# DixianZhu/deBWT

Measured on AMD Instinct MI355X. Metric: Gbp/sec BWT build (30 Gbp synthetic DNA); bit-exact vs CPU ref; 1/2/4/8-GPU, higher is better.
Workload: dtype u64

## Files before the change

debwt_amd/_lib.py:

```python
import ctypes
import os
import subprocess

_HERE = os.path.dirname(os.path.abspath(__file__))
LIB_PATH = os.environ.get("DEBWT_HIP_LIB", os.path.join(_HERE, "libdebwt_hip.so"))
_lib = None


class DebwtConfig(ctypes.Structure):
    _fields_ = [("k", ctypes.c_int), ("device", ctypes.c_int), ("sort_algo", ctypes.c_int),
                ("reserved", ctypes.c_int)]


class DebwtPackedText(ctypes.Structure):
    _fields_ = [("words", ctypes.POINTER(ctypes.c_uint64)), ("nwords", ctypes.c_uint64), ("n", ctypes.c_uint64),
                ("sep", ctypes.POINTER(ctypes.c_uint64)), ("nrec", ctypes.c_uint64),
                ("seconds_read", ctypes.c_double), ("seconds_pack", ctypes.c_double)]


class DebwtStats(ctypes.Structure):
    _fields_ = ([(n, ctypes.c_uint64) for n in (
        "n", "nrec", "red_capacity", "blue_capacity", "blue_bound_num", "case3num", "sp_len",
        "special_branch_num", "n_main", "distinct_keys", "blue_large_blocks", "blue_max_block")] +
        [(n, ctypes.c_float) for n in (
# ... 265 lines not shown


class DebwtMultiStats(ctypes.Structure):
    _fields_ = [("n", ctypes.c_uint64), ("nrec", ctypes.c_uint64), ("ngpus", ctypes.c_uint32), ("rounds", ctypes.c_uint32),
                ("key_bytes_in", ctypes.c_uint64), ("blue_bytes_in", ctypes.c_uint64), ("ms_build", ctypes.c_float),
                ("key_mode", ctypes.c_uint32), ("exchange_backend", ctypes.c_uint32)]

    def as_dict(self):
        return {n: getattr(self, n) for n, _ in self._fields_}


SYMBOLS = [
    "debwt_create", "debwt_destroy", "debwt_strerror", "debwt_last_error", "debwt_load_text",
    "debwt_load_ascii", "debwt_kmer_sort_rle", "debwt_classify", "debwt_sp_generate", "debwt_blue_sort",
    "debwt_bwt_assemble", "debwt_build", "debwt_fetch_bwt", "debwt_bwt_device_ptr", "debwt_get_stats",
    "debwt_fetch_array", "debwt_kmer_count_sorted", "debwt_radix_sort_u64", "debwt_radix_sort_u64_range", "debwt_radix_pair_passes", "debwt_radix_bucket_passes", "debwt_radix_low_finishes", "debwt_verify_inverse",
    "debwt_shard_begin", "debwt_shard_histogram", "debwt_shard_set_range", "debwt_shard_classify_local",
    "debwt_shard_facts_export", "debwt_shard_classify_global", "debwt_shard_info", "debwt_shard_fetch",
    "debwt_shard_partition_keys", "debwt_shard_plan", "debwt_shard_ranges", "debwt_shard_sort_begin",
    "debwt_shard_sort_range", "debwt_shard_sort_end", "debwt_concat_rows", "debwt_shard_export", "debwt_census_words", "debwt_shard_sp_flags", "debwt_shard_sp_emit",
    "debwt_shard_sp_import", "debwt_shard_blue_route", "debwt_shard_blue_place", "debwt_set_range_cap", "debwt_pack_fasta", "debwt_free_packed", "debwt_load_fasta", "debwt_pack_fasta_opts", "debwt_load_fasta_opts", "debwt_fasta_text_bound", "debwt_host_release_hold", "debwt_special_digest", "debwt_bwt_census", "debwt_fetch_rows", "debwt_verify_device", "debwt_multi_create", "debwt_multi_destroy", "debwt_multi_last_error",
    "debwt_multi_load_text", "debwt_multi_load_fasta", "debwt_multi_build", "debwt_multi_fetch_bwt", "debwt_multi_get_stats",
    "debwt_multi_verify", "debwt_multi_shard", "debwt_pinned_alloc", "debwt_pinned_free", "debwt_shard_key_mode",
    "debwt_multi_set_key_mode", "debwt_special_compare", "debwt_build_to_host", "debwt_multi_set_exchange", "debwt_reserve",
    "debwt_multi_set_serial", "debwt_multi_get_shard_report", "debwt_multi_step_name", "debwt_get_config",
    "debwt_dump_reference_files", "debwt_shard_scratch",
    "debwt_fm_create", "debwt_fm_open", "debwt_fm_last_error", "debwt_fm_info_get", "debwt_fm_samples",
    "debwt_fm_record_starts", "debwt_fm_count", "debwt_fm_locate", "debwt_fm_destroy",
    "debwt_fm_search", "debwt_fm_search_stats_get", "debwt_fm_mems", "debwt_fm_mems_stats_get",
    "debwt_fm_attach_text", "debwt_fm_extend", "debwt_fm_extend_stats_get", "debwt_fm_cluster_seeds",
    "debwt_fm_map_defaults", "debwt_fm_map", "debwt_fm_map_stats_get",
# ... 59 lines not shown
    L.debwt_bwt_device_ptr.argtypes = [vp, ctypes.POINTER(vp)]
    L.debwt_get_stats.restype = ctypes.c_int
    L.debwt_get_stats.argtypes = [vp, ctypes.POINTER(DebwtStats)]
    L.debwt_fetch_array.restype = ctypes.c_int
    L.debwt_fetch_array.argtypes = [vp, ctypes.c_int, vp, ctypes.c_uint64, u64p]
    L.debwt_kmer_count_sorted.restype = ctypes.c_int
    L.debwt_kmer_count_sorted.argtypes = [vp, u64p, u64p, ctypes.c_uint64, u64p]
    L.debwt_radix_sort_u64.restype = ctypes.c_int
    L.debwt_radix_sort_u64.argtypes = [vp, vp, vp, ctypes.c_uint64, ctypes.c_int, ctypes.POINTER(ctypes.c_float)]
    L.debwt_radix_pair_passes.restype = ctypes.c_uint64
    L.debwt_radix_pair_passes.argtypes = []
    L.debwt_radix_bucket_passes.restype = ctypes.c_uint64
    L.debwt_radix_bucket_passes.argtypes = []
    L.debwt_radix_low_finishes.restype = ctypes.c_uint64
    L.debwt_radix_low_finishes.argtypes = []
    L.debwt_radix_sort_u64_range.restype = ctypes.c_int
    L.debwt_radix_sort_u64_range.argtypes = [vp, vp, vp, ctypes.c_uint64, ctypes.c_int, ctypes.c_uint64, ctypes.c_uint64,
                                             ctypes.POINTER(ctypes.c_float)]
    L.debwt_verify_inverse.restype = ctypes.c_int
    L.debwt_verify_inverse.argtypes = [u64p, ctypes.c_uint64, u64p, ctypes.c_uint64, ctypes.c_uint64,
                                       ctypes.POINTER(ctypes.c_uint8)]
    L.debwt_shard_begin.restype = ctypes.c_int
    L.debwt_shard_begin.argtypes = [vp, ctypes.c_int, ctypes.c_int]
    L.debwt_shard_histogram.restype = ctypes.c_int
    L.debwt_shard_histogram.argtypes = [vp, u64p]
    L.debwt_shard_set_range.restype = ctypes.c_int
    L.debwt_shard_set_range.argtypes = [vp, ctypes.c_uint32, ctypes.c_uint32, ctypes.c_uint64, ctypes.c_uint64]
    L.debwt_shard_classify_local.restype = ctypes.c_int
    L.debwt_shard_classify_local.argtypes = [vp, u64p, u64p, u64p]
    L.debwt_shard_facts_export.restype = ctypes.c_int
# ... 237 lines not shown
```

debwt_amd/csrc/debwt_hip.hip:

```cpp
#include "../../include/debwt_hip.h"

#include <hip/hip_runtime.h>

#include <algorithm>
#include <new>
#include <chrono>
#include <cmath>
#include <cstdio>
#include <cstring>
#include <atomic>
#include <string>
#include <thread>
#include <tuple>
#include <vector>

#include "radix_sort.h"
#include "special_host.h"
#include "fasta_host.h"
#include "gz_parallel.h"
#include "stage_kernels.h"
#include "special_kernels.h"
#include "verify_kernels.h"
#include "fm_kernels.h"
#include "fm_search_kernels.h"
// ... 83 lines not shown
    u64 *routed = nullptr;
    struct SubSlice { u64 g0, g1, S, B; };
    std::vector<SubSlice> sub;
    std::thread special_thread;
    bool special_running = false;
    u64 g0 = 0, g1 = 0;
    u64 S_local = 0, B_slice = 0, sp_off = 0;
    int hbits = 10, pbits = 13;
    bool mzfilter = false;
    int mzw = 16;
    bool mztable = false;
    bool abs32 = true;

    hipStream_t copy_stream = nullptr;
    hipEvent_t ev_copy = nullptr, ev_copy2 = nullptr;
    std::vector<u64> census;
    bool census_valid = false;
    hipEvent_t ev[8]{};
    hipEvent_t ev_pass[16][2]{};
    int n_pass_events = 0;
};

namespace {

#define HIPCHK(ctx, call)                                                                      \
    do {                                                                                       \
        hipError_t e_ = (call);                                                                \
        if (e_ != hipSuccess) {                                                                \
            (ctx)->err = std::string(#call) + ": " + hipGetErrorString(e_);                    \
            return e_ == hipErrorOutOfMemory ? DEBWT_ENOMEM : DEBWT_EDEVICE;                   \
        }                                                                                      \
    } while (0)

size_t reclaim(debwt_ctx *c, const DevBuf *keep) {
    if (!c->reclaim_ok) return 0;
    std::vector<DevBuf *> idle;
    if (c->stage >= ST_CLASSIFIED) {
        idle = {&c->keysB, &c->dk, &c->dstart, &c->rs_rle, &c->pflag};
        if (!c->exchange) idle.push_back(&c->keysA);
        c->sk = nullptr; c->routed = nullptr;
    } else {
        idle = {&c->htab, &c->mi_list, &c->qlist, &c->qwave, &c->blue_tmp, &c->ls_buf, &c->vidx, &c->vtmp, &c->large_k0,
                &c->large_en, &c->rowsym, &c->spn, &c->spsym, &c->rbits, &c->blue, &c->momask, &c->mimask};
    }
    size_t freed = 0;
    (void)hipStreamSynchronize(c->stream);
    for (DevBuf *b : idle)
        if (b != keep && b->p) { freed += b->cap; (void)hipFree(b->p); b->p = nullptr; b->cap = 0; }
    if (getenv("DEBWT_TRACE_ALLOC")) fprintf(stderr, "reclaim: %.2f GB of idle buffers released\n", freed / 1e9);
    return freed;
}

int ensure(debwt_ctx *c, DevBuf &b, size_t bytes) {
    if (bytes <= b.cap) return DEBWT_OK;
    static const bool trace = getenv("DEBWT_TRACE_ALLOC") != nullptr;
    const auto t0 = std::chrono::steady_clock::now();
    const size_t old = b.cap;
    if (b.p) { HIPCHK(c, hipStreamSynchronize(c->stream)); HIPCHK(c, hipFree(b.p)); b.p = nullptr; b.cap = 0; }
    const auto t1 = std::chrono::steady_clock::now();
    size_t want = bytes + bytes / 16 + 256;
    hipError_t me = hipMalloc(&b.p, want);
// ... 72 lines not shown
int sync_check(debwt_ctx *c) {
    HIPCHK(c, hipStreamSynchronize(c->stream));
    HIPCHK(c, hipGetLastError());
    return DEBWT_OK;
}

struct DrainOnError {
    debwt_ctx *c;
    bool armed = true;
    ~DrainOnError() {
        if (!armed) return;
        if (c->copy_stream) (void)hipStreamSynchronize(c->copy_stream);
        if (c->stream) (void)hipStreamSynchronize(c->stream);
    }
};

inline u32 grid_for(u64 n, u32 block) { return (u32)((n + block - 1) / block); }

RadixWorkspace radix_ws(debwt_ctx *c) {
    RadixWorkspace ws{};
    ws.counts = c->rs_counts.as<u32>();
    ws.over = c->rs_over.as<u32>();
    ws.h_over = c->h_over;
    ws.over_cap = c->rs_over.cap >= 48 ? (u32)std::min<size_t>((c->rs_over.cap - 32) / 16, 0xFFFFFFFFu) : 0;
    ws.skew_list = c->rs_skew.as<u32>();
    ws.pair = c->rs_pair.as<u32>();
    ws.pair_cap = c->rs_pair.cap;
    return ws;
}

// ... 21 lines not shown
}

}


static std::vector<DevBuf *> all_buffers(debwt_ctx *c) {
    return {&c->text, &c->sepbits, &c->sep, &c->keysA, &c->keysB, &c->rs_counts, &c->cp_counts, &c->dk,
            &c->dstart, &c->mchar, &c->head_keys, &c->facts, &c->facts_tmp, &c->red, &c->red_q,
            &c->mi_j0, &c->mi_freq, &c->bstart, &c->cursor, &c->blue, &c->spkey, &c->sprow, &c->spchr,
            &c->branch, &c->pflag, &c->spsym, &c->spn, &c->bwt, &c->hmask, &c->hash_rows, &c->dollar,
            &c->large_q, &c->large_k0, &c->large_en, &c->rowsym, &c->momask, &c->mimask, &c->rbits, &c->rs_over, &c->rs_skew, &c->rs_pair,
            &c->mi_list, &c->htab, &c->fact_work, &c->facts_all, &c->shard_hist, &c->dest_tab, &c->qbounds, &c->qcursor,
            &c->sx, &c->sppos, &c->sprec, &c->tail_d, &c->brbits,
            &c->blk_j0, &c->blk_freq, &c->blk_start, &c->facts_acc, &c->large_tmp, &c->blue_tmp, &c->sub_start, &c->sub_j0,
            &c->sub_freq, &c->sub_depth, &c->range_hist, &c->rs_rle, &c->ls_buf, &c->vidx, &c->vtmp, &c->qlist, &c->qwave,
            &c->blue_done};
}

extern "C" const char *debwt_strerror(int code) {
    switch (code) {
        case DEBWT_OK: return "ok";
        case DEBWT_EINVAL: return "invalid argument";
        case DEBWT_ENOMEM: return "out of memory";
        case DEBWT_EDEVICE: return "HIP runtime error";
        case DEBWT_ESTATE: return "stage called out of order";
        case DEBWT_ERANGE: return "input exceeds a capacity of this build";
        case DEBWT_EINTERNAL: return "internal consistency check failed";
        case DEBWT_EIO: return "file could not be written";
        default: return "unknown error";
    }
}
// ... 7 lines not shown
}

extern "C" int debwt_create(const debwt_config *cfg, debwt_ctx **out) {
    if (!cfg || !out || cfg->k < 12 || cfg->k > 32) return DEBWT_EINVAL;
    int ndev = 0;
    if (hipGetDeviceCount(&ndev) != hipSuccess || cfg->device < 0 || cfg->device >= ndev) return DEBWT_EDEVICE;
    debwt_ctx *c = new (std::nothrow) debwt_ctx();
    if (!c) return DEBWT_ENOMEM;
    c->cfg = *cfg;
    if (c->cfg.sort_algo == 0) c->cfg.sort_algo = 3;
    c->K = cfg->k - 1;
    int rc = DEBWT_OK;
    auto fail = [&](int code) { debwt_destroy(c); return code; };
    if (hipSetDevice(cfg->device) != hipSuccess) return fail(DEBWT_EDEVICE);
    if (hipStreamCreateWithFlags(&c->stream, hipStreamNonBlocking) != hipSuccess) return fail(DEBWT_EDEVICE);
    if (hipHostMalloc((void **)&c->h_scalars, 64 * sizeof(u32), hipHostMallocDefault) != hipSuccess)
        return fail(DEBWT_ENOMEM);
    for (auto &e : c->ev) if (hipEventCreate(&e) != hipSuccess) return fail(DEBWT_EDEVICE);
    for (auto &p : c->ev_pass) for (auto &e : p) if (hipEventCreate(&e) != hipSuccess) return fail(DEBWT_EDEVICE);
    if ((rc = ensure(c, c->rs_counts, radix_workspace_bytes(0))) != DEBWT_OK) return fail(rc);
    if ((rc = ensure(c, c->rs_over, radix_over_bytes(1 << 20))) != DEBWT_OK) return fail(rc);
    if (hipHostMalloc((void **)&c->h_over, 64, hipHostMallocDefault) != hipSuccess)
        return fail(DEBWT_ENOMEM);
    if ((rc = ensure(c, c->cp_counts, 8 * (CP_MAXCHUNKS + 16) * sizeof(u32))) != DEBWT_OK) return fail(rc);
    if ((rc = ensure(c, c->dollar, 64)) != DEBWT_OK) return fail(rc);
    *out = c;
    return DEBWT_OK;
}

extern "C" void debwt_destroy(debwt_ctx *c) {
    if (!c) return;
    if (c->special_running) { c->special_thread.join(); c->special_running = false; }
    (void)hipSetDevice(c->cfg.device);
    if (c->stream) (void)hipStreamSynchronize(c->stream);
    for (DevBuf *b : all_buffers(c)) if (b->p) (void)hipFree(b->p);
    if (c->h_scalars) (void)hipHostFree(c->h_scalars);
    if (c->h_over) (void)hipHostFree(c->h_over);
    for (auto &e : c->ev) if (e) (void)hipEventDestroy(e);
    for (auto &p : c->ev_pass) for (auto &e : p) if (e) (void)hipEventDestroy(e);
    if (c->ev_copy) (void)hipEventDestroy(c->ev_copy);
    if (c->ev_copy2) (void)hipEventDestroy(c->ev_copy2);
    if (c->copy_stream) { (void)hipStreamSynchronize(c->copy_stream); (void)hipStreamDestroy(c->copy_stream); }
    if (c->stream) (void)hipStreamDestroy(c->stream);
    delete c;
}

static void join_special(debwt_ctx *c);

extern "C" int debwt_load_text(debwt_ctx *c, const uint64_t *packed, uint64_t n, const uint64_t *sep, uint64_t nrec) {
    if (!c || !packed || !sep || nrec == 0 || n < 34) return DEBWT_EINVAL;
    join_special(c);
    if (sep[nrec - 1] != n - 1) return DEBWT_EINVAL;
    uint64_t prev = 0;
    for (uint64_t r = 0; r < nrec; r++) {
        uint64_t start = r ? sep[r - 1] + 1 : 0;
        if (sep[r] < start + 33 || sep[r] >= n) return DEBWT_EINVAL;
        prev = sep[r];
// ... 778 lines not shown
    ENSURE(c, c->htab, ht_slots * sizeof(HSlot));
    HIPCHK(c, hipMemsetAsync(c->rbits.p, 0, rb_bytes, c->stream));
    HIPCHK(c, hipMemsetAsync(c->htab.p, 0, ht_slots * sizeof(HSlot), c->stream));
    if (c->R) {
        k_build_hash<<<grid_for(c->R, 256), 256, 0, c->stream>>>(c->red.as<u64>(), c->R, c->red_q.as<u32>(),
                                                                c->blk_start.as<u64>(), c->abs32 ? 1 : 0, (u32)c->qbase,
                                                                (u32)c->Q, hbits, c->htab.as<HSlot>(), c->mzfilter ? 0 : pb,
                                                                c->rbits.as<u32>(), c->mztable ? c->K : 0);
        if (c->mzfilter)
            k_build_mzfilter<<<grid_for(c->R, 256), 256, 0, c->stream>>>(c->red.as<u64>(), c->R, c->K, pb, c->rbits.as<u64>(), c->mzw);
    }
    return DEBWT_OK;
}

#define SP_SLICE_GROUPS (1ull << 26)
static SpBlockIds sp_block_ids(debwt_ctx *c) {
    if (!c->route_direct) return SpBlockIds{nullptr, nullptr, nullptr, 0};
    return SpBlockIds{c->qlist.as<u32>(), c->qwave.as<unsigned long long>(), c->qwave.as<u64>() + 1, c->gq0};
}
static int sp_block_ids_begin(debwt_ctx *c, u64 gq0, u64 groups) {
    c->route_direct = true; c->gq0 = gq0;
    ENSURE(c, c->qlist, (std::min<u64>(groups * 32, c->Btotal) + 64) * 4);
    ENSURE(c, c->qwave, ((groups + 63) / 64 + 2) * 8);
    HIPCHK(c, hipMemsetAsync(c->qwave.p, 0, 8, c->stream));
    return DEBWT_OK;
}

static int sp_flags(debwt_ctx *c, u64 g0, u64 g1) {
    int rc;
    if (g1 - g0 > (1ull << 27) - 2) { c->err = "text slice of the SP stage exceeds 2^32 positions"; return DEBWT_ERANGE; }
    c->g0 = g0; c->g1 = g1;
    const u64 ng = g1 - g0;
    if (ng && c->mzfilter && c->mztable)
        k_sp_flags<2><<<grid_for(ng, DEBWT_BLOCK), DEBWT_BLOCK, 0, c->stream>>>(
            c->text.as<u64>(), c->sepbits.as<u64>(), c->n, c->K, c->htab.as<HSlot>(), c->hbits, c->rbits.as<u32>(), c->pbits,
            c->branch.as<u64>(), c->nbranch, c->momask.as<u32>(), c->mimask.as<u32>(), g0, g1,
            sp_block_ids(c), c->branch_bitmap ? c->brbits.as<u64>() : nullptr);
    else if (ng && c->mzfilter)
        k_sp_flags<1><<<grid_for(ng, DEBWT_BLOCK), DEBWT_BLOCK, 0, c->stream>>>(
            c->text.as<u64>(), c->sepbits.as<u64>(), c->n, c->K, c->htab.as<HSlot>(), c->hbits, c->rbits.as<u32>(), c->pbits,
            c->branch.as<u64>(), c->nbranch, c->momask.as<u32>(), c->mimask.as<u32>(), g0, g1,
            sp_block_ids(c), c->branch_bitmap ? c->brbits.as<u64>() : nullptr, c->mzw);
    else if (ng)
        k_sp_flags<0><<<grid_for(ng, DEBWT_BLOCK), DEBWT_BLOCK, 0, c->stream>>>(
            c->text.as<u64>(), c->sepbits.as<u64>(), c->n, c->K, c->htab.as<HSlot>(), c->hbits, c->rbits.as<u32>(), c->pbits,
            c->branch.as<u64>(), c->nbranch, c->momask.as<u32>(), c->mimask.as<u32>(), g0, g1,
            sp_block_ids(c), c->branch_bitmap ? c->brbits.as<u64>() : nullptr);
    SpCountF fc{c->momask.as<u32>() + g0, c->mimask.as<u32>() + g0};
    if ((rc = cp_count2(c, fc, ng, cp_area(c, 0), 8, cp_area(c, 1), 10))) return rc;
    if ((rc = sync_check(c))) return rc;
    c->S_local = c->h_scalars[8];
    c->B_slice = c->h_scalars[10];
    return DEBWT_OK;
}

static int sp_emit(debwt_ctx *c, u64 sp_off, u64 *routed = nullptr, int qshift = 0) {
    const u64 ng = c->g1 - c->g0;
    c->sp_off = sp_off;
    ENSURE_KEEP(c, c->spsym, sp_off + c->S_local + 64, c->shard_world > 1 ? 0 : sp_off);
    if (!routed) ENSURE(c, c->mi_list, c->B_slice * 16 + 64);
    if (ng) {
        SpEmitArgs ea{c->text.as<u64>(), c->sepbits.as<u64>(), c->n, c->K, c->momask.as<u32>(), c->mimask.as<u32>(),
                      c->spsym.as<u8>(), routed ? nullptr : c->mi_list.as<ulonglong2>(), c->g0, sp_off,
                      routed, qshift, sp_block_ids(c)};
        u32 nchunks; u64 chunk;
        plan_chunks(ng, &nchunks, &chunk);
        k_sp_emit<<<nchunks, DEBWT_BLOCK, 0, c->stream>>>(ea, ng, chunk, cp_area(c, 0), cp_area(c, 1));
    }
    return DEBWT_OK;
}

static int sp_finish(debwt_ctx *c, u64 S) {
    c->S = S;
    u64 ntriples = (S >> 6) + 3;
    ENSURE(c, c->spn, ntriples * 24);
    k_pack_sp<<<grid_for(ntriples, 256), 256, 0, c->stream>>>(c->spsym.as<u8>(), S, ntriples, c->spn.as<u64>());
    c->st.sp_len = S;
    c->stage = ST_SP;
    return DEBWT_OK;
}

extern "C" int debwt_sp_generate(debwt_ctx *c) {
// ... 14 lines not shown
                            !((c->cfg.reserved & 262144) && c->ranges.size() > 1);
    const size_t P = c->ranges.size();
    bool route_ranges = !route_sort && c->shard_world == 1 && P > 1 && P <= RS_RADIX && c->Q > 0 && c->n < (1ull << (qshift - 3)) &&
                        !(c->cfg.reserved & 32);
    for (size_t i = 0; route_ranges && i < P; i++) route_ranges = c->ranges[i].B < 0xFFFFFFF0ull - (1ull << 20);
    std::vector<u64> rfill(P, 0), roffs(P + 1, 0);
    if (route_ranges) {
        std::vector<u32> qb(P + 1);
        for (size_t i = 0; i < P; i++) qb[i] = (u32)c->ranges[i].qbase;
        qb[P] = (u32)c->Q;
        ENSURE(c, c->qbounds, (P + 1) * 4);
        HIPCHK(c, hipMemcpyAsync(c->qbounds.p, qb.data(), (P + 1) * 4, hipMemcpyHostToDevice, c->stream));
        HIPCHK(c, hipStreamSynchronize(c->stream));
    }
    c->route_direct = false;
    for (u64 g0 = 0; g0 < ngroups; g0 += slice_groups) {
        const u64 g1 = std::min(ngroups, g0 + slice_groups);
        if ((route_sort || route_ranges) && (rc = sp_block_ids_begin(c, g0, g1 - g0))) return rc;
        if ((rc = sp_flags(c, g0, g1))) return rc;
        if (route_sort) {
            if (Bseen + c->B_slice > c->B) { c->err = "multi-in positions exceed the block total"; return DEBWT_EINTERNAL; }
            if ((rc = sp_emit(c, S, c->blue.as<u64>() + Bseen, qshift))) return rc;
        } else if (route_ranges) {
            u64 *ta = c->keysA.as<u64>(), *tb = c->keysB.as<u64>();
            size_t tb_cap = c->keysB.cap / 8;
            if (c->keysA.cap < c->B_slice * 8 + 64) { ENSURE(c, c->blue_tmp, c->B_slice * 8 + 64); ta = c->blue_tmp.as<u64>(); }
            if (c->keysB.cap < c->B_slice * 8 + 64) { ENSURE(c, c->mi_list, c->B_slice * 8 + 64); tb = c->mi_list.as<u64>(); tb_cap = c->mi_list.cap / 8; }
            if ((rc = sp_emit(c, S, ta, qshift))) return rc;
            if (c->B_slice) {
                ENSURE(c, c->rs_over, radix_over_bytes(c->B_slice));
                RsDigit dg{};
// ... 218 lines not shown
}

static int blue_sort_part(debwt_ctx *c, const BlueQueue &bq, u64 q0, u64 nq, u64 l0, u64 nl) {
    int rc;
    if (!nq) return DEBWT_OK;
    const u32 Q = (u32)nq;
    const u64 *bst = c->blk_start.as<u64>() + q0, *bj0 = c->blk_j0.as<u64>() + q0;
    const u32 *bfr = c->blk_freq.as<u32>() + q0;
    const BlueSub &sub = bq.sub;
    const u32 sub_cap = bq.cap;
    u32 *sub_count = bq.count;
    HIPCHK(c, hipMemsetAsync(c->sub_freq.p, 0, (size_t)sub_cap * 4, c->stream));
    HIPCHK(c, hipMemsetAsync(sub_count, 0, 4, c->stream));
    BlueSub none{};
    u32 g1 = (u32)std::min<u64>(Q, 1u << 16);
    const u32 tiny = (c->cfg.reserved & 16777216) ? 0u : 2 * BLUE_TINY;
    if (tiny) {
        k_blue_tiny<16><<<g1, 64, 0, c->stream>>>(c->blue.as<u64>(), bst, bfr, bj0, Q, c->spn.as<u64>(), c->S, c->mchar.as<u8>(),
                                                  nullptr, nullptr);
        k_blue_tiny<32><<<g1, 64, 0, c->stream>>>(c->blue.as<u64>(), bst, bfr, bj0, Q, c->spn.as<u64>(), c->S, c->mchar.as<u8>(),
                                                  nullptr, nullptr);
    }
    k_blue_refine<64, 128, 0><<<g1, 64, 0, c->stream>>>(c->blue.as<u64>(), bst, bfr, bj0, Q, tiny,
                                                       c->spn.as<u64>(), c->S, c->mchar.as<u8>(), nullptr, nullptr, none);
    k_blue_refine<64, 256, 128><<<g1, 64, 0, c->stream>>>(c->blue.as<u64>(), bst, bfr, bj0, Q, 128u, c->spn.as<u64>(), c->S,
                                                         c->mchar.as<u8>(), nullptr, nullptr, sub);
    const bool split1024 = c->n1024 >= 1024;
    const bool by_classes = split1024 || c->n512 >= 1024;
    const u8 *done = nullptr;
    if ((by_classes || (c->cfg.reserved & 1048576)) && sub.cap && !(c->cfg.reserved & 524288)) {
        ENSURE(c, c->blue_done, c->Q + 64);
        u8 *dn = c->blue_done.as<u8>() + q0;
        HIPCHK(c, hipMemsetAsync(dn, 0, Q, c->stream));
        const u32 gc = (u32)std::min<u64>(Q, 1u << 14);
        k_blue_classify<BLUE_WAVE_CAP, BLUE_WAVE_CAP><<<gc, 256, 0, c->stream>>>(c->blue.as<u64>(), bst, bfr, bj0, Q, 256u, c->spn.as<u64>(),
                                                                                 c->S, c->mchar.as<u8>(), sub, dn);
        k_blue_classify<1024, BLUE_WAVE_CAP><<<gc, 256, 0, c->stream>>>(c->blue.as<u64>(), bst, bfr, bj0, Q, (u32)BLUE_WAVE_CAP,
                                                                        c->spn.as<u64>(), c->S, c->mchar.as<u8>(), sub, dn);
        k_blue_classify<BLUE_LDS_CAP, BLUE_WAVE_CAP><<<(u32)std::min<u64>(Q, 1u << 12), 256, 0, c->stream>>>(
            c->blue.as<u64>(), bst, bfr, bj0, Q, 1024u, c->spn.as<u64>(), c->S, c->mchar.as<u8>(), sub, dn);
        done = dn;
    }
    k_blue_refine<256, BLUE_WAVE_CAP, 128><<<(u32)std::min<u64>(Q, 1u << 14), 256, 0, c->stream>>>(
        c->blue.as<u64>(), bst, bfr, bj0, Q, 256u, c->spn.as<u64>(), c->S, c->mchar.as<u8>(), nullptr, nullptr, sub, done);
    u32 g2 = (u32)std::min<u64>(Q, 1u << 12);
    if (split1024)
        k_blue_refine<256, 1024, BLUE_WAVE_CAP><<<g2, 256, 0, c->stream>>>(c->blue.as<u64>(), bst, bfr, bj0, Q, (u32)BLUE_WAVE_CAP,
                                                                      c->spn.as<u64>(), c->S, c->mchar.as<u8>(), nullptr, nullptr, sub, done);
    k_blue_refine<256, BLUE_LDS_CAP, BLUE_WAVE_CAP><<<g2, 256, 0, c->stream>>>(c->blue.as<u64>(), bst, bfr, bj0, Q,
                                                                  split1024 ? 1024u : (u32)BLUE_WAVE_CAP, c->spn.as<u64>(), c->S,
                                                                  c->mchar.as<u8>(), nullptr, nullptr, sub, done);
    if (nl && (rc = sort_large_blocks(c, sub, l0, nl))) return rc;
    const u32 gs = std::min<u32>(sub_cap, 1u << 16);
    if (done) {
        u32 *snap = sub_count + 1;
        for (int level = 0; level < BLUE_QUEUE_LEVELS; level++) {
            k_copy_u32<<<1, 1, 0, c->stream>>>(sub_count, snap);
            k_blue_classify<BLUE_WAVE_CAP, BLUE_WAVE_CAP><<<std::min<u32>(gs, 1u << 14), 256, 0, c->stream>>>(
                c->blue.as<u64>(), c->sub_start.as<u64>(), c->sub_freq.as<u32>(), c->sub_j0.as<u64>(), sub_cap, 128u, c->spn.as<u64>(),
                c->S, c->mchar.as<u8>(), sub, nullptr, c->sub_depth.as<u32>(), snap, c->sub_freq.as<u32>());
        }
    }
    if (tiny) {
        k_blue_tiny<16><<<gs, 64, 0, c->stream>>>(c->blue.as<u64>(), c->sub_start.as<u64>(), c->sub_freq.as<u32>(), c->sub_j0.as<u64>(),
                                                  sub_cap, c->spn.as<u64>(), c->S, c->mchar.as<u8>(), c->sub_depth.as<u32>(), sub_count);
        k_blue_tiny<32><<<gs, 64, 0, c->stream>>>(c->blue.as<u64>(), c->sub_start.as<u64>(), c->sub_freq.as<u32>(), c->sub_j0.as<u64>(),
// ... 796 lines not shown
        std::vector<u32> first(D);
        HIPCHK(c, hipMemcpy(first.data(), c->dstart.p, D * 4, hipMemcpyDeviceToHost));
        for (u64 i = 0; i < ncopy; i++) counts[i] = (i + 1 < D ? first[i + 1] : (u32)Mk) - first[i];
    }
    return DEBWT_OK;
}

extern "C" int debwt_radix_sort_u64(debwt_ctx *c, uint64_t *d_keys, uint64_t *d_tmp, uint64_t count, int key_bits,
                                    float *ms_per_pass) {
    return debwt_radix_sort_u64_range(c, d_keys, d_tmp, count, key_bits, 0, 0, ms_per_pass);
}

extern "C" uint64_t debwt_radix_pair_passes(void) { return radix_pair_passes(); }
extern "C" uint64_t debwt_radix_bucket_passes(void) { return radix_bucket_passes(); }
extern "C" uint64_t debwt_radix_low_finishes(void) { return radix_low_finishes(); }

__global__ void k_keys_outside(const u64 *__restrict__ keys, u64 n, u64 lo, u64 hi, u32 *__restrict__ flag) {
    bool bad = false;
    for (u64 i = (u64)blockIdx.x * blockDim.x + threadIdx.x; i < n; i += (u64)gridDim.x * blockDim.x) bad |= keys[i] < lo || keys[i] > hi;
    if (bad) *flag = 1u;
}

extern "C" int debwt_radix_sort_u64_range(debwt_ctx *c, uint64_t *d_keys, uint64_t *d_tmp, uint64_t count, int key_bits,
                                          uint64_t key_lo, uint64_t key_hi, float *ms_per_pass) {
    if (!c || !d_keys || !d_tmp || key_bits < 1 || key_bits > 64) return DEBWT_EINVAL;
    if (key_hi && key_hi <= key_lo) return DEBWT_EINVAL;
    if (count >= 0xFFFFFFF0ull) return DEBWT_ERANGE;
    HIPCHK(c, hipSetDevice(c->cfg.device));
    ENSURE(c, c->rs_skew, (count / 2048 + 2) * 4);
    ENSURE(c, c->rs_over, radix_over_bytes(count));
// ... 4209 lines not shown
```

include/debwt_hip.h:

```cpp
#ifndef DEBWT_HIP_H
#define DEBWT_HIP_H
#include <stddef.h>
#include <stdint.h>
#ifdef __cplusplus
extern "C" {
#endif

#define DEBWT_OK 0
#define DEBWT_EINVAL (-1)
#define DEBWT_ENOMEM (-2)
#define DEBWT_EDEVICE (-3)
#define DEBWT_ESTATE (-4)
#define DEBWT_ERANGE (-5)
#define DEBWT_EINTERNAL (-6)
#define DEBWT_EIO (-7)

typedef struct debwt_ctx debwt_ctx;

typedef struct {
    int k;
    int device;
    int sort_algo;
    int reserved;
} debwt_config;
// ... 161 lines not shown
#define DEBWT_DUMP_BLOCKS 2
#define DEBWT_DUMP_SP 3
int debwt_dump_reference_files(debwt_ctx *ctx, const char *dir, int stage);


int debwt_kmer_count_sorted(debwt_ctx *ctx, uint64_t *kmers, uint64_t *counts, uint64_t capacity,
                            uint64_t *distinct);

int debwt_radix_sort_u64(debwt_ctx *ctx, uint64_t *d_keys, uint64_t *d_tmp, uint64_t count, int key_bits,
                         float *ms_per_pass);
int debwt_radix_sort_u64_range(debwt_ctx *ctx, uint64_t *d_keys, uint64_t *d_tmp, uint64_t count, int key_bits,
                               uint64_t key_lo, uint64_t key_hi, float *ms_per_pass);
uint64_t debwt_radix_pair_passes(void);
uint64_t debwt_radix_bucket_passes(void);
uint64_t debwt_radix_low_finishes(void);

int debwt_special_digest(const uint64_t *packed, uint64_t n, const uint64_t *sep, uint64_t nrec, int k, uint64_t digest[4]);

int debwt_special_compare(debwt_ctx *ctx, uint64_t mismatch[6]);

int debwt_verify_inverse(const uint64_t *bwt, uint64_t n, const uint64_t *hash_rows, uint64_t nrec,
                         uint64_t dollar_row, uint8_t *sym_out);

typedef struct {
    uint64_t segments, steps, mismatches, broken_links, search_failures, search_steps;
    float ms_index, ms_search, ms_walk;
    int ok;
} debwt_verify_report;
int debwt_verify_device(debwt_ctx *ctx, const uint64_t *d_words, const uint64_t *hash_rows, uint64_t dollar_row,
                        uint64_t segments, debwt_verify_report *report);
// ... 295 lines not shown
```

Before: 24.36.

## Overlap SP flag/emit slices and small blue-block refinement on an auxiliary stream

Adds an auxiliary HIP stream with fork/join events. The SP stage now double-buffers its per-slice block-id and count areas, so the flags of slice s+1 are computed on the main stream while slice s is emitted on the aux stream. The blue sort launches the tiny/small-block refinement kernels on the aux stream concurrently with the large-class classify/refine kernels on the main stream. The aim is to hide host sync gaps and let underutilizing small kernels run alongside each other, at the cost of extra buffers, more events, and some risk of races on shared sub-block counters.

```diff
diff --git a/debwt_amd/_lib.py b/debwt_amd/_lib.py
--- a/debwt_amd/_lib.py
+++ b/debwt_amd/_lib.py
@@ -303,7 +303,7 @@
     "debwt_create", "debwt_destroy", "debwt_strerror", "debwt_last_error", "debwt_load_text",
     "debwt_load_ascii", "debwt_kmer_sort_rle", "debwt_classify", "debwt_sp_generate", "debwt_blue_sort",
     "debwt_bwt_assemble", "debwt_build", "debwt_fetch_bwt", "debwt_bwt_device_ptr", "debwt_get_stats",
-    "debwt_fetch_array", "debwt_kmer_count_sorted", "debwt_radix_sort_u64", "debwt_radix_sort_u64_range", "debwt_radix_pair_passes", "debwt_radix_bucket_passes", "debwt_radix_low_finishes", "debwt_verify_inverse",
+    "debwt_fetch_array", "debwt_kmer_count_sorted", "debwt_radix_sort_u64", "debwt_radix_sort_u64_range", "debwt_radix_pair_passes", "debwt_radix_bucket_passes", "debwt_radix_low_finishes", "debwt_overlapped_launches", "debwt_verify_inverse",
     "debwt_shard_begin", "debwt_shard_histogram", "debwt_shard_set_range", "debwt_shard_classify_local",
     "debwt_shard_facts_export", "debwt_shard_classify_global", "debwt_shard_info", "debwt_shard_fetch",
     "debwt_shard_partition_keys", "debwt_shard_plan", "debwt_shard_ranges", "debwt_shard_sort_begin",
@@ -393,6 +393,8 @@
     L.debwt_radix_bucket_passes.argtypes = []
     L.debwt_radix_low_finishes.restype = ctypes.c_uint64
     L.debwt_radix_low_finishes.argtypes = []
+    L.debwt_overlapped_launches.restype = ctypes.c_uint64
+    L.debwt_overlapped_launches.argtypes = []
     L.debwt_radix_sort_u64_range.restype = ctypes.c_int
     L.debwt_radix_sort_u64_range.argtypes = [vp, vp, vp, ctypes.c_uint64, ctypes.c_int, ctypes.c_uint64, ctypes.c_uint64,
                                              ctypes.POINTER(ctypes.c_float)]
diff --git a/debwt_amd/csrc/debwt_hip.hip b/debwt_amd/csrc/debwt_hip.hip
--- a/debwt_amd/csrc/debwt_hip.hip
+++ b/debwt_amd/csrc/debwt_hip.hip
@@ -121,6 +121,12 @@
 
     hipStream_t copy_stream = nullptr;
     hipEvent_t ev_copy = nullptr, ev_copy2 = nullptr;
+    hipStream_t aux_stream = nullptr;
+    hipEvent_t ev_fork = nullptr, ev_join = nullptr, ev_totals[2]{}, ev_emit[2]{};
+    bool aux_busy = false;
+    DevBuf qwave2, qlist2;
+    u32 *qlist_b = nullptr;
+    u64 gq0_b = 0;
     std::vector<u64> census;
     bool census_valid = false;
     hipEvent_t ev[8]{};
@@ -147,11 +153,12 @@
         if (!c->exchange) idle.push_back(&c->keysA);
         c->sk = nullptr; c->routed = nullptr;
     } else {
-        idle = {&c->htab, &c->mi_list, &c->qlist, &c->qwave, &c->blue_tmp, &c->ls_buf, &c->vidx, &c->vtmp, &c->large_k0,
+        idle = {&c->htab, &c->mi_list, &c->qlist, &c->qwave, &c->qlist2, &c->qwave2, &c->blue_tmp, &c->ls_buf, &c->vidx, &c->vtmp, &c->large_k0,
                 &c->large_en, &c->rowsym, &c->spn, &c->spsym, &c->rbits, &c->blue, &c->momask, &c->mimask};
     }
     size_t freed = 0;
     (void)hipStreamSynchronize(c->stream);
+    if (c->aux_stream) (void)hipStreamSynchronize(c->aux_stream);
     for (DevBuf *b : idle)
         if (b != keep && b->p) { freed += b->cap; (void)hipFree(b->p); b->p = nullptr; b->cap = 0; }
     if (getenv("DEBWT_TRACE_ALLOC")) fprintf(stderr, "reclaim: %.2f GB of idle buffers released\n", freed / 1e9);
@@ -254,6 +261,39 @@
         if (c->stream) (void)hipStreamSynchronize(c->stream);
     }
 };
+
+enum { STREAMS_SP = 1, STREAMS_BLUE = 2 };
+std::atomic<u64> overlapped_launches{0};
+int streams_parts(const debwt_ctx *c) {
+    if (!c->aux_stream) return 0;
+    const char *e = getenv("DEBWT_STREAMS");
+    if (!e || !*e) return STREAMS_SP | STREAMS_BLUE;
+    if (!strcmp(e, "sp")) return STREAMS_SP;
+    if (!strcmp(e, "blue")) return STREAMS_BLUE;
+    return atoi(e) == 1 ? 0 : STREAMS_SP | STREAMS_BLUE;
+}
+int aux_fork(debwt_ctx *c) {
+    HIPCHK(c, hipEventRecord(c->ev_fork, c->stream));
+    HIPCHK(c, hipStreamWaitEvent(c->aux_stream, c->ev_fork, 0));
+    c->aux_busy = true;
+    return DEBWT_OK;
+}
+int aux_join(debwt_ctx *c) {
+    if (!c->aux_busy) return DEBWT_OK;
+    HIPCHK(c, hipEventRecord(c->ev_join, c->aux_stream));
+    HIPCHK(c, hipStreamWaitEvent(c->stream, c->ev_join, 0));
+    c->aux_busy = false;
+    return DEBWT_OK;
+}
+struct AuxDrain {
+    debwt_ctx *c;
+    ~AuxDrain() {
+        if (!c->aux_busy) return;
+        (void)hipStreamSynchronize(c->aux_stream);
+        c->aux_busy = false;
+    }
+};
+inline void aux_count(u64 n = 1) { overlapped_launches.fetch_add(n, std::memory_order_relaxed); }
 
 inline u32 grid_for(u64 n, u32 block) { return (u32)((n + block - 1) / block); }
 
@@ -305,7 +345,7 @@
             &c->sx, &c->sppos, &c->sprec, &c->tail_d, &c->brbits,
             &c->blk_j0, &c->blk_freq, &c->blk_start, &c->facts_acc, &c->large_tmp, &c->blue_tmp, &c->sub_start, &c->sub_j0,
             &c->sub_freq, &c->sub_depth, &c->range_hist, &c->rs_rle, &c->ls_buf, &c->vidx, &c->vtmp, &c->qlist, &c->qwave,
-            &c->blue_done};
+            &c->blue_done, &c->qwave2, &c->qlist2};
 }
 
 extern "C" const char *debwt_strerror(int code) {
@@ -343,6 +383,9 @@
     auto fail = [&](int code) { debwt_destroy(c); return code; };
     if (hipSetDevice(cfg->device) != hipSuccess) return fail(DEBWT_EDEVICE);
     if (hipStreamCreateWithFlags(&c->stream, hipStreamNonBlocking) != hipSuccess) return fail(DEBWT_EDEVICE);
+    if (hipStreamCreateWithFlags(&c->aux_stream, hipStreamNonBlocking) != hipSuccess) return fail(DEBWT_EDEVICE);
+    for (hipEvent_t *e : {&c->ev_fork, &c->ev_join, &c->ev_totals[0], &c->ev_totals[1], &c->ev_emit[0], &c->ev_emit[1]})
+        if (hipEventCreateWithFlags(e, hipEventDisableTiming) != hipSuccess) return fail(DEBWT_EDEVICE);
     if (hipHostMalloc((void **)&c->h_scalars, 64 * sizeof(u32), hipHostMallocDefault) != hipSuccess)
         return fail(DEBWT_ENOMEM);
     for (auto &e : c->ev) if (hipEventCreate(&e) != hipSuccess) return fail(DEBWT_EDEVICE);
@@ -351,7 +394,7 @@
     if ((rc = ensure(c, c->rs_over, radix_over_bytes(1 << 20))) != DEBWT_OK) return fail(rc);
     if (hipHostMalloc((void **)&c->h_over, 64, hipHostMallocDefault) != hipSuccess)
         return fail(DEBWT_ENOMEM);
-    if ((rc = ensure(c, c->cp_counts, 8 * (CP_MAXCHUNKS + 16) * sizeof(u32))) != DEBWT_OK) return fail(rc);
+    if ((rc = ensure(c, c->cp_counts, 10 * (CP_MAXCHUNKS + 16) * sizeof(u32))) != DEBWT_OK) return fail(rc);
     if ((rc = ensure(c, c->dollar, 64)) != DEBWT_OK) return fail(rc);
     *out = c;
     return DEBWT_OK;
@@ -362,6 +405,7 @@
     if (c->special_running) { c->special_thread.join(); c->special_running = false; }
     (void)hipSetDevice(c->cfg.device);
     if (c->stream) (void)hipStreamSynchronize(c->stream);
+    if (c->aux_stream) (void)hipStreamSynchronize(c->aux_stream);
     for (DevBuf *b : all_buffers(c)) if (b->p) (void)hipFree(b->p);
     if (c->h_scalars) (void)hipHostFree(c->h_scalars);
     if (c->h_over) (void)hipHostFree(c->h_over);
@@ -370,6 +414,8 @@
     if (c->ev_copy) (void)hipEventDestroy(c->ev_copy);
     if (c->ev_copy2) (void)hipEventDestroy(c->ev_copy2);
     if (c->copy_stream) { (void)hipStreamSynchronize(c->copy_stream); (void)hipStreamDestroy(c->copy_stream); }
+    for (hipEvent_t e : {c->ev_fork, c->ev_join, c->ev_totals[0], c->ev_totals[1], c->ev_emit[0], c->ev_emit[1]}) if (e) (void)hipEventDestroy(e);
+    if (c->aux_stream) (void)hipStreamDestroy(c->aux_stream);
     if (c->stream) (void)hipStreamDestroy(c->stream);
     delete c;
 }
@@ -1178,47 +1224,63 @@
 }
 
 #define SP_SLICE_GROUPS (1ull << 26)
-static SpBlockIds sp_block_ids(debwt_ctx *c) {
+static SpBlockIds sp_block_ids(debwt_ctx *c, int set = 0) {
     if (!c->route_direct) return SpBlockIds{nullptr, nullptr, nullptr, 0};
+    if (set) return SpBlockIds{c->qlist_b, c->qwave2.as<unsigned long long>(), c->qwave2.as<u64>() + 1, c->gq0_b};
     return SpBlockIds{c->qlist.as<u32>(), c->qwave.as<unsigned long long>(), c->qwave.as<u64>() + 1, c->gq0};
 }
-static int sp_block_ids_begin(debwt_ctx *c, u64 gq0, u64 groups) {
-    c->route_direct = true; c->gq0 = gq0;
-    ENSURE(c, c->qlist, (std::min<u64>(groups * 32, c->Btotal) + 64) * 4);
+static size_t sp_block_ids_bytes(const debwt_ctx *c, u64 groups) { return (std::min<u64>(groups * 32, c->Btotal) + 64) * 4; }
+static int sp_block_ids_begin(debwt_ctx *c, u64 gq0, u64 groups, int set = 0) {
+    c->route_direct = true;
+    if (set) {
+        c->gq0_b = gq0;
+        ENSURE(c, c->qwave2, ((groups + 63) / 64 + 2) * 8);
+        HIPCHK(c, hipMemsetAsync(c->qwave2.p, 0, 8, c->stream));
+        return DEBWT_OK;
+    }
+    c->gq0 = gq0;
+    ENSURE(c, c->qlist, sp_block_ids_bytes(c, groups));
     ENSURE(c, c->qwave, ((groups + 63) / 64 + 2) * 8);
     HIPCHK(c, hipMemsetAsync(c->qwave.p, 0, 8, c->stream));
     return DEBWT_OK;
 }
 
-static int sp_flags(debwt_ctx *c, u64 g0, u64 g1) {
-    int rc;
+static u32 *sp_area(debwt_ctx *c, int set, int which) { return cp_area(c, (set ? 8 : 0) + which); }
+static int sp_slot(int set, int which) { return set ? 40 + which : 8 + 2 * which; }
+
+static int sp_flags_queue(debwt_ctx *c, u64 g0, u64 g1, int set) {
     if (g1 - g0 > (1ull << 27) - 2) { c->err = "text slice of the SP stage exceeds 2^32 positions"; return DEBWT_ERANGE; }
-    c->g0 = g0; c->g1 = g1;
     const u64 ng = g1 - g0;
     if (ng && c->mzfilter && c->mztable)
         k_sp_flags<2><<<grid_for(ng, DEBWT_BLOCK), DEBWT_BLOCK, 0, c->stream>>>(
             c->text.as<u64>(), c->sepbits.as<u64>(), c->n, c->K, c->htab.as<HSlot>(), c->hbits, c->rbits.as<u32>(), c->pbits,
             c->branch.as<u64>(), c->nbranch, c->momask.as<u32>(), c->mimask.as<u32>(), g0, g1,
-            sp_block_ids(c), c->branch_bitmap ? c->brbits.as<u64>() : nullptr);
+            sp_block_ids(c, set), c->branch_bitmap ? c->brbits.as<u64>() : nullptr);
     else if (ng && c->mzfilter)
         k_sp_flags<1><<<grid_for(ng, DEBWT_BLOCK), DEBWT_BLOCK, 0, c->stream>>>(
             c->text.as<u64>(), c->sepbits.as<u64>(), c->n, c->K, c->htab.as<HSlot>(), c->hbits, c->rbits.as<u32>(), c->pbits,
             c->branch.as<u64>(), c->nbranch, c->momask.as<u32>(), c->mimask.as<u32>(), g0, g1,
-            sp_block_ids(c), c->branch_bitmap ? c->brbits.as<u64>() : nullptr, c->mzw);
+            sp_block_ids(c, set), c->branch_bitmap ? c->brbits.as<u64>() : nullptr, c->mzw);
     else if (ng)
         k_sp_flags<0><<<grid_for(ng, DEBWT_BLOCK), DEBWT_BLOCK, 0, c->stream>>>(
             c->text.as<u64>(), c->sepbits.as<u64>(), c->n, c->K, c->htab.as<HSlot>(), c->hbits, c->rbits.as<u32>(), c->pbits,
             c->branch.as<u64>(), c->nbranch, c->momask.as<u32>(), c->mimask.as<u32>(), g0, g1,
-            sp_block_ids(c), c->branch_bitmap ? c->brbits.as<u64>() : nullptr);
+            sp_block_ids(c, set), c->branch_bitmap ? c->brbits.as<u64>() : nullptr);
     SpCountF fc{c->momask.as<u32>() + g0, c->mimask.as<u32>() + g0};
-    if ((rc = cp_count2(c, fc, ng, cp_area(c, 0), 8, cp_area(c, 1), 10))) return rc;
+    return cp_count2(c, fc, ng, sp_area(c, set, 0), sp_slot(set, 0), sp_area(c, set, 1), sp_slot(set, 1));
+}
+
+static int sp_flags(debwt_ctx *c, u64 g0, u64 g1) {
+    int rc;
+    c->g0 = g0; c->g1 = g1;
+    if ((rc = sp_flags_queue(c, g0, g1, 0))) return rc;
     if ((rc = sync_check(c))) return rc;
-    c->S_local = c->h_scalars[8];
-    c->B_slice = c->h_scalars[10];
-    return DEBWT_OK;
-}
-
-static int sp_emit(debwt_ctx *c, u64 sp_off, u64 *routed = nullptr, int qshift = 0) {
+    c->S_local = c->h_scalars[sp_slot(0, 0)];
+    c->B_slice = c->h_scalars[sp_slot(0, 1)];
+    return DEBWT_OK;
+}
+
+static int sp_emit(debwt_ctx *c, u64 sp_off, u64 *routed = nullptr, int qshift = 0, int set = 0, bool aux = false) {
     const u64 ng = c->g1 - c->g0;
     c->sp_off = sp_off;
     ENSURE_KEEP(c, c->spsym, sp_off + c->S_local + 64, c->shard_world > 1 ? 0 : sp_off);
@@ -1226,10 +1288,11 @@
     if (ng) {
         SpEmitArgs ea{c->text.as<u64>(), c->sepbits.as<u64>(), c->n, c->K, c->momask.as<u32>(), c->mimask.as<u32>(),
                       c->spsym.as<u8>(), routed ? nullptr : c->mi_list.as<ulonglong2>(), c->g0, sp_off,
-                      routed, qshift, sp_block_ids(c)};
+                      routed, qshift, sp_block_ids(c, set)};
         u32 nchunks; u64 chunk;
         plan_chunks(ng, &nchunks, &chunk);
-        k_sp_emit<<<nchunks, DEBWT_BLOCK, 0, c->stream>>>(ea, ng, chunk, cp_area(c, 0), cp_area(c, 1));
+        k_sp_emit<<<nchunks, DEBWT_BLOCK, 0, aux ? c->aux_stream : c->stream>>>(ea, ng, chunk, sp_area(c, set, 0), sp_area(c, set, 1));
+        if (aux) aux_count();
     }
     return DEBWT_OK;
 }
@@ -1274,7 +1337,47 @@
         HIPCHK(c, hipStreamSynchronize(c->stream));
     }
     c->route_direct = false;
-    for (u64 g0 = 0; g0 < ngroups; g0 += slice_groups) {
+    AuxDrain drain{c};
+    bool pipelined = route_sort && (streams_parts(c) & STREAMS_SP) && !c->exchange;
+    if (pipelined) {
+        const size_t need = sp_block_ids_bytes(c, std::min(ngroups, slice_groups));
+        if (c->keysB.cap >= need) c->qlist_b = c->keysB.as<u32>();
+        else if (c->keysA.cap >= need) c->qlist_b = c->keysA.as<u32>();
+        else if (need <= ((size_t)64 << 20)) { ENSURE(c, c->qlist2, need); c->qlist_b = c->qlist2.as<u32>(); }
+        else pipelined = false;
+    }
+    if (pipelined) {
+        const u64 nslices = (ngroups + slice_groups - 1) / slice_groups;
+        auto queue_flags = [&](u64 s) -> int {
+            const int set = (int)(s & 1);
+            const u64 a = s * slice_groups, b = std::min(ngroups, a + slice_groups);
+            if (s >= 2) HIPCHK(c, hipStreamWaitEvent(c->stream, c->ev_emit[set], 0));
+            int r;
+            if ((r = sp_block_ids_begin(c, a, b - a, set))) return r;
+            if ((r = sp_flags_queue(c, a, b, set))) return r;
+            HIPCHK(c, hipEventRecord(c->ev_totals[set], c->stream));
+            return DEBWT_OK;
+        };
+        if ((rc = queue_flags(0))) return rc;
+        for (u64 s = 0; s < nslices; s++) {
+            const int set = (int)(s & 1);
+            if (s + 1 < nslices && (rc = queue_flags(s + 1))) return rc;
+            HIPCHK(c, hipEventSynchronize(c->ev_totals[set]));
+            HIPCHK(c, hipGetLastError());
+            c->g0 = s * slice_groups; c->g1 = std::min(ngroups, c->g0 + slice_groups);
+            c->S_local = c->h_scalars[sp_slot(set, 0)];
+            c->B_slice = c->h_scalars[sp_slot(set, 1)];
+            if (Bseen + c->B_slice > c->B) { c->err = "multi-in positions exceed the block total"; return DEBWT_EINTERNAL; }
+            if (c->spsym.cap < S + c->S_local + 64) HIPCHK(c, hipStreamSynchronize(c->aux_stream));
+            HIPCHK(c, hipStreamWaitEvent(c->aux_stream, c->ev_totals[set], 0));
+            c->aux_busy = true;
+            if ((rc = sp_emit(c, S, c->blue.as<u64>() + Bseen, qshift, set, true))) return rc;
+            HIPCHK(c, hipEventRecord(c->ev_emit[set], c->aux_stream));
+            S += c->S_local; Bseen += c->B_slice;
+        }
+        if ((rc = aux_join(c))) return rc;
+    }
+    for (u64 g0 = 0; !pipelined && g0 < ngroups; g0 += slice_groups) {
         const u64 g1 = std::min(ngroups, g0 + slice_groups);
         if ((route_sort || route_ranges) && (rc = sp_block_ids_begin(c, g0, g1 - g0))) return rc;
         if ((rc = sp_flags(c, g0, g1))) return rc;
@@ -1523,35 +1626,28 @@
     HIPCHK(c, hipMemsetAsync(sub_count, 0, 4, c->stream));
     BlueSub none{};
     u32 g1 = (u32)std::min<u64>(Q, 1u << 16);
-    const u32 tiny = (c->cfg.reserved & 16777216) ? 0u : 2 * BLUE_TINY;
-    if (tiny) {
-        k_blue_tiny<16><<<g1, 64, 0, c->stream>>>(c->blue.as<u64>(), bst, bfr, bj0, Q, c->spn.as<u64>(), c->S, c->mchar.as<u8>(),
-                                                  nullptr, nullptr);
-        k_blue_tiny<32><<<g1, 64, 0, c->stream>>>(c->blue.as<u64>(), bst, bfr, bj0, Q, c->spn.as<u64>(), c->S, c->mchar.as<u8>(),
-                                                  nullptr, nullptr);
-    }
-    k_blue_refine<64, 128, 0><<<g1, 64, 0, c->stream>>>(c->blue.as<u64>(), bst, bfr, bj0, Q, tiny,
-                                                       c->spn.as<u64>(), c->S, c->mchar.as<u8>(), nullptr, nullptr, none);
-    k_blue_refine<64, 256, 128><<<g1, 64, 0, c->stream>>>(c->blue.as<u64>(), bst, bfr, bj0, Q, 128u, c->spn.as<u64>(), c->S,
-                                                         c->mchar.as<u8>(), nullptr, nullptr, sub);
     const bool split1024 = c->n1024 >= 1024;
     const bool by_classes = split1024 || c->n512 >= 1024;
-    const u8 *done = nullptr;
+    u8 *done = nullptr;
     if ((by_classes || (c->cfg.reserved & 1048576)) && sub.cap && !(c->cfg.reserved & 524288)) {
         ENSURE(c, c->blue_done, c->Q + 64);
-        u8 *dn = c->blue_done.as<u8>() + q0;
-        HIPCHK(c, hipMemsetAsync(dn, 0, Q, c->stream));
-        const u32 gc = (u32)std::min<u64>(Q, 1u << 14);
-        k_blue_classify<BLUE_WAVE_CAP, BLUE_WAVE_CAP><<<gc, 256, 0, c->stream>>>(c->blue.as<u64>(), bst, bfr, bj0, Q, 256u, c->spn.as<u64>(),
-                                                                                 c->S, c->mchar.as<u8>(), sub, dn);
+        done = c->blue_done.as<u8>() + q0;
+        HIPCHK(c, hipMemsetAsync(done, 0, Q, c->stream));
+    }
+    AuxDrain drain{c};
+    const bool fork = (streams_parts(c) & STREAMS_BLUE) != 0;
+    hipStream_t ks = c->stream;
+    if (fork) {
+        if ((rc = aux_fork(c))) return rc;
+        ks = c->aux_stream;
+    }
+    const u32 gc = (u32)std::min<u64>(Q, 1u << 14);
+    if (done) {
         k_blue_classify<1024, BLUE_WAVE_CAP><<<gc, 256, 0, c->stream>>>(c->blue.as<u64>(), bst, bfr, bj0, Q, (u32)BLUE_WAVE_CAP,
-                                                                        c->spn.as<u64>(), c->S, c->mchar.as<u8>(), sub, dn);
+                                                                        c->spn.as<u64>(), c->S, c->mchar.as<u8>(), sub, done);
         k_blue_classify<BLUE_LDS_CAP, BLUE_WAVE_CAP><<<(u32)std::min<u64>(Q, 1u << 12), 256, 0, c->stream>>>(
-            c->blue.as<u64>(), bst, bfr, bj0, Q, 1024u, c->spn.as<u64>(), c->S, c->mchar.as<u8>(), sub, dn);
-        done = dn;
-    }
-    k_blue_refine<256, BLUE_WAVE_CAP, 128><<<(u32)std::min<u64>(Q, 1u << 14), 256, 0, c->stream>>>(
-        c->blue.as<u64>(), bst, bfr, bj0, Q, 256u, c->spn.as<u64>(), c->S, c->mchar.as<u8>(), nullptr, nullptr, sub, done);
+            c->blue.as<u64>(), bst, bfr, bj0, Q, 1024u, c->spn.as<u64>(), c->S, c->mchar.as<u8>(), sub, done);
+    }
     u32 g2 = (u32)std::min<u64>(Q, 1u << 12);
     if (split1024)
         k_blue_refine<256, 1024, BLUE_WAVE_CAP><<<g2, 256, 0, c->stream>>>(c->blue.as<u64>(), bst, bfr, bj0, Q, (u32)BLUE_WAVE_CAP,
@@ -1559,6 +1655,24 @@
     k_blue_refine<256, BLUE_LDS_CAP, BLUE_WAVE_CAP><<<g2, 256, 0, c->stream>>>(c->blue.as<u64>(), bst, bfr, bj0, Q,
                                                                   split1024 ? 1024u : (u32)BLUE_WAVE_CAP, c->spn.as<u64>(), c->S,
                                                                   c->mchar.as<u8>(), nullptr, nullptr, sub, done);
+    const u32 tiny = (c->cfg.reserved & 16777216) ? 0u : 2 * BLUE_TINY;
+    if (tiny) {
+        k_blue_tiny<16><<<g1, 64, 0, ks>>>(c->blue.as<u64>(), bst, bfr, bj0, Q, c->spn.as<u64>(), c->S, c->mchar.as<u8>(),
+                                          nullptr, nullptr);
+        k_blue_tiny<32><<<g1, 64, 0, ks>>>(c->blue.as<u64>(), bst, bfr, bj0, Q, c->spn.as<u64>(), c->S, c->mchar.as<u8>(),
+                                          nullptr, nullptr);
+    }
+    k_blue_refine<64, 128, 0><<<g1, 64, 0, ks>>>(c->blue.as<u64>(), bst, bfr, bj0, Q, tiny,
+                                               c->spn.as<u64>(), c->S, c->mchar.as<u8>(), nullptr, nullptr, none);
+    k_blue_refine<64, 256, 128><<<g1, 64, 0, ks>>>(c->blue.as<u64>(), bst, bfr, bj0, Q, 128u, c->spn.as<u64>(), c->S,
+                                                 c->mchar.as<u8>(), nullptr, nullptr, sub);
+    if (done)
+        k_blue_classify<BLUE_WAVE_CAP, BLUE_WAVE_CAP><<<gc, 256, 0, ks>>>(c->blue.as<u64>(), bst, bfr, bj0, Q, 256u, c->spn.as<u64>(),
+                                                                         c->S, c->mchar.as<u8>(), sub, done);
+    k_blue_refine<256, BLUE_WAVE_CAP, 128><<<gc, 256, 0, ks>>>(
+        c->blue.as<u64>(), bst, bfr, bj0, Q, 256u, c->spn.as<u64>(), c->S, c->mchar.as<u8>(), nullptr, nullptr, sub, done);
+    if (fork) aux_count((tiny ? 2 : 0) + (done ? 4 : 3));
+    if ((rc = aux_join(c))) return rc;
     if (nl && (rc = sort_large_blocks(c, sub, l0, nl))) return rc;
     const u32 gs = std::min<u32>(sub_cap, 1u << 16);
     if (done) {
@@ -2385,6 +2499,7 @@
 extern "C" uint64_t debwt_radix_pair_passes(void) { return radix_pair_passes(); }
 extern "C" uint64_t debwt_radix_bucket_passes(void) { return radix_bucket_passes(); }
 extern "C" uint64_t debwt_radix_low_finishes(void) { return radix_low_finishes(); }
+extern "C" uint64_t debwt_overlapped_launches(void) { return overlapped_launches.load(std::memory_order_relaxed); }
 
 __global__ void k_keys_outside(const u64 *__restrict__ keys, u64 n, u64 lo, u64 hi, u32 *__restrict__ flag) {
     bool bad = false;
diff --git a/include/debwt_hip.h b/include/debwt_hip.h
--- a/include/debwt_hip.h
+++ b/include/debwt_hip.h
@@ -199,6 +199,7 @@
 uint64_t debwt_radix_pair_passes(void);
 uint64_t debwt_radix_bucket_passes(void);
 uint64_t debwt_radix_low_finishes(void);
+uint64_t debwt_overlapped_launches(void);
 
 int debwt_special_digest(const uint64_t *packed, uint64_t n, const uint64_t *sep, uint64_t nrec, int k, uint64_t digest[4]);
 
```

Result: no change. 24.49 (median of 6 runs) (+0.5%).
